# google/libultrahdr

Hardware: AMD Instinct MI355X
Metric: Mpixels/s encode+decode (API-1 P010+YUV420, 4K), device-resident round trip (higher is better)
Workload: dtype f32; 1 GPU; API-1 3840x2160 round trip per step: encode (P010 HLG + YCbCr420 -> two-pass 3-ch gain map at scale 1, FDCT q95, Huffman: two JPEG scans) + decode (Huffman, IDCT, applyGainMap -> RGBA_F16 linear); frames resident in HBM

## Files before the change

### libultrahdr_amd/csrc/api_context.cpp

```cpp
#include "api_internal.h"

#include <sys/mman.h>
#include <mutex>
#include <algorithm>

namespace uhdr_api {
uhdr_error_info_t ensure(DeviceBuf& b, size_t bytes) {
  if (b.cap >= bytes) return ok_status();
  if (b.p) (void)hipFree(b.p);
  b.p = nullptr;
  b.cap = 0;
  size_t want = bytes + (bytes >> 3) + 256;
  HIP_TRY(hipMalloc(&b.p, want));
  b.cap = want;
  return ok_status();
}


size_t bytes_per_sample(int fmt) {
  switch (fmt) {
    case UHDR_IMG_FMT_24bppYCbCrP010:
    case UHDR_IMG_FMT_30bppYCbCr444: return 2;
    case UHDR_IMG_FMT_24bppRGB888: return 3;
    case UHDR_IMG_FMT_32bppRGBA8888:
// ... 507 lines not shown
  int n = 0;
  if (hipGetDeviceCount(&n) != hipSuccess) return 0;
  return n;
}

int uhdr_hip_current_device(void) {
  int d = -1;
  if (hipGetDevice(&d) != hipSuccess) return -1;
  return d;
}

uhdr_hip_ctx_t* uhdr_hip_create(int device, uhdr_error_info_t* err) {
  auto fail = [&](const char* what, hipError_t e) -> uhdr_hip_ctx_t* {
    if (err) *err = err_status(UHDR_CODEC_ERROR, "uhdr_hip_create: %s failed: %s (no CPU fallback exists behind this library)",
                               what, hipGetErrorString(e));
    return nullptr;
  };
  if (err) *err = ok_status();
  int n = 0;
  hipError_t e = hipGetDeviceCount(&n);
  if (e != hipSuccess || n == 0) return fail("hipGetDeviceCount", e == hipSuccess ? hipErrorNoDevice : e);
  if (device < 0) {
    e = hipGetDevice(&device);
    if (e != hipSuccess) return fail("hipGetDevice", e);
  }
  if (device >= n) return fail("device index", hipErrorInvalidDevice);
  e = hipSetDevice(device);
  if (e != hipSuccess) return fail("hipSetDevice", e);
  uhdr_hip_ctx* c = new uhdr_hip_ctx();
  c->device = device;
  {
    const char* e = getenv("UHDR_HIP_HUFF_TWO_PASS");
    c->huff_two_pass = e && atoi(e) != 0;
    e = getenv("UHDR_HIP_HUFF_ROUTE_LOG");
    c->huff_route_log = e && atoi(e) != 0;
  }
  e = hipStreamCreateWithFlags(&c->own_stream, hipStreamNonBlocking);
  if (e != hipSuccess) { delete c; return fail("hipStreamCreate", e); }
  c->stream = c->own_stream;
  uhdr_error_info_t st = upload_lut(&c->d_srgb, host::srgb_inv_oetf_lut(), c->stream);
  if (st.error_code != UHDR_CODEC_OK) {
    if (err) *err = st;
    (void)hipStreamDestroy(c->own_stream);
    delete c;
    return nullptr;
  }
  return c;
}

void uhdr_hip_destroy(uhdr_hip_ctx_t* c) {
  if (!c) return;
  (void)hipSetDevice(c->device);
  (void)hipStreamSynchronize(c->stream);
  for (auto& e : c->prof_entries) { (void)hipEventDestroy(e.a); (void)hipEventDestroy(e.b); }
  float* luts[] = {c->d_srgb, c->d_hlg_inv, c->d_pq_inv, c->d_hlg_oetf, c->d_pq_oetf, c->d_hlg_inv_ootf, (float*)c->d_math,
                   c->d_hlg_buckets, c->d_pq_buckets, c->d_hlg_buckets_pre, c->d_pq_buckets_pre};
  for (float* p : luts) if (p) (void)hipFree(p);
  for (int i = 0; i < kTableSlots; i++) {
    if (c->h_tab[i]) (void)hipHostFree(c->h_tab[i]);
    if (c->d_tab[i]) (void)hipFree(c->d_tab[i]);
    if (c->tab_ev[i]) (void)hipEventDestroy(c->tab_ev[i]);
  }
  for (auto& b : c->scratch) if (b.p) (void)hipFree(b.p);
  for (auto& b : c->jpg) if (b.p) (void)hipFree(b.p);
  for (auto& b : c->enc) if (b.p) (void)hipFree(b.p);
  if (c->huff_slots.p) (void)hipFree(c->huff_slots.p);
// ... 274 lines not shown
```

### libultrahdr_amd/csrc/api_entropy.cpp

```cpp
#include "api_internal.h"

#include <condition_variable>
#include <functional>
#include <mutex>

uhdr_error_info_t uhdr_api::check_scan(const uhdr_hip_jpeg_scan_t* sc, bool need_coef, int* mcus_per_row, int* mcu_rows, int* blocks_per_mcu) {
  if (!sc) return err_status(UHDR_CODEC_INVALID_PARAM, "received nullptr for the scan description");
  if (sc->num_components != 1 && sc->num_components != 3)
    return err_status(UHDR_CODEC_INVALID_PARAM, "a scan has 1 or 3 components, received %d", sc->num_components);
  if (sc->w == 0 || sc->h == 0 || sc->w > 65535 || sc->h > 65535)
    return err_status(UHDR_CODEC_INVALID_PARAM, "image dimensions %ux%u are outside JPEG's 1..65535", sc->w, sc->h);
  int hmax = 1, vmax = 1, bpm = 0;
  for (int i = 0; i < sc->num_components; i++) {
    const int hs = sc->num_components == 1 ? 1 : sc->h_samp[i], vs = sc->num_components == 1 ? 1 : sc->v_samp[i];
    if (hs < 1 || hs > 2 || vs < 1 || vs > 2) return err_status(UHDR_CODEC_INVALID_PARAM, "component %d: sampling factors %dx%d not in {1, 2}", i, hs, vs);
    if (hs > hmax) hmax = hs;
    if (vs > vmax) vmax = vs;
    bpm += hs * vs;
    if (need_coef && (!sc->coef[i] || ((uintptr_t)sc->coef[i] & 15)))
      return err_status(UHDR_CODEC_INVALID_PARAM, "coefficient buffer %d is null or not 16-byte aligned", i);
    if (sc->blocks_w[i] < 1 || sc->blocks_h[i] < 1) return err_status(UHDR_CODEC_INVALID_PARAM, "component %d: empty block grid", i);
  }
  if (sc->num_components == 1) {
    *mcus_per_row = sc->blocks_w[0];
// ... 40 lines not shown
  const bool stream = sc->restart_interval == 0;
  if (!stream && (sc->restart_interval < 1 || sc->restart_interval > 65535 || sc->restart_interval * bpm > 64))
    return err_status(UHDR_CODEC_UNSUPPORTED_FEATURE, "restart_interval must be 0 (no markers) or in 1..%d for %d blocks per MCU (one wavefront "
                      "encodes one restart interval of at most 64 blocks); received %d", 64 / bpm, bpm, sc->restart_interval);
  if (stream && 2 * bpm > 64) return err_status(UHDR_CODEC_UNSUPPORTED_FEATURE, "%d blocks per MCU: outside the HIP path", bpm);
  HIP_TRY(hipSetDevice(c->device));
  if (!c->d_huff) {
    std::vector<uint32_t> blob(host::jpeg_huff_code_tables());
    blob.resize((size_t)host::kHuffTabWords + 16);
    memcpy(blob.data() + host::kHuffTabWords, host::jpeg_zigzag_to_natural(), 64);
    HIP_TRY(hipMalloc((void**)&c->d_huff, blob.size() * sizeof(uint32_t)));
    HIP_TRY(hipMemcpyAsync(c->d_huff, blob.data(), blob.size() * sizeof(uint32_t), hipMemcpyHostToDevice, c->stream));
    HIP_TRY(hipStreamSynchronize(c->stream));
  }
  HuffArgs a;
  memset(&a, 0, sizeof a);
  a.ncomp = sc->num_components;
  for (int i = 0; i < a.ncomp; i++) {
    a.coef[i] = sc->coef[i];
    a.bw[i] = sc->blocks_w[i]; a.bh[i] = sc->blocks_h[i];
    a.hs[i] = a.ncomp == 1 ? 1 : sc->h_samp[i]; a.vs[i] = a.ncomp == 1 ? 1 : sc->v_samp[i];
  }
  a.mcus_per_row = mpr;
  a.total_mcus = mpr * mrows;
  a.ri = stream ? huff_stream_segment_mcus(bpm) : sc->restart_interval;
  a.blocks_per_mcu = bpm;
  a.nseg = (a.total_mcus + a.ri - 1) / a.ri;
  a.tables = c->d_huff;
  a.zigzag = (const uint8_t*)(c->d_huff + host::kHuffTabWords);
  if (stream) {
    if (out_capacity > 0xFFFFFFF0u) out_capacity = 0xFFFFFFF0u;
    HuffStream t;
    memset(&t, 0, sizeof t);
    t.raw_words = ((uint64_t)out_capacity + 3) / 4 + 1;
    const uint64_t worst_words = (uint64_t)a.total_mcus * bpm * 52 + 2;
    if (t.raw_words > worst_words) t.raw_words = worst_words;
    const int nchunks = huff_stuff_chunks(t.raw_words * 4u);
    UHDR_TRY(ensure(c->scratch[4], (size_t)t.raw_words * 4));
    UHDR_TRY(ensure(c->scratch[5], ((size_t)a.nseg + 2) * sizeof(uint64_t) + (4 + (size_t)a.nseg + (size_t)nchunks) * sizeof(uint32_t)));
    t.raw = (uint32_t*)c->scratch[4].p;
    t.seg_start = (uint64_t*)c->scratch[5].p;
    uint64_t* d_total = t.seg_start + (size_t)a.nseg + 1;
    t.meta = (uint32_t*)(d_total + 1);
    t.seg_bits = t.meta + 4;
    uint32_t* chunk_counts = t.seg_bits + a.nseg;
    if (!c->huff_two_pass) {
      const size_t need = huff_stream_slot_bytes(a.nseg);
      if (c->huff_slots.cap >= need || !c->huff_slots_refused || need < c->huff_slots_refused) {
        if (ensure(c->huff_slots, need).error_code == UHDR_CODEC_OK) {
          t.slots = (uint32_t*)c->huff_slots.p;
        } else {
          (void)hipGetLastError();
          c->huff_slots_refused = need;
          fprintf(stderr, "uhdr_hip: no device memory for %zu bytes of Huffman segment slots: marker-less scans of that size take the two-pass route\n", need);
        }
      }
    }
    if (c->huff_route_log) fprintf(stderr, "uhdr_hip: huffman_encode stream route=%s nseg=%d\n", t.slots ? "one_walk" : "two_pass", a.nseg);
    {
      ProfScope ps(c, "huffman_encode");
      HIP_TRY(launch_huffman_encode_stream(a, t, chunk_counts, d_total, out, (uint64_t)out_capacity, c->stream));
    }
    c->stats.entropy_encode_stream++;
    if (!c->h_flags) HIP_TRY(hipHostMalloc((void**)&c->h_flags, 64 * sizeof(uint32_t), hipHostMallocDefault));
    uint32_t* hp = c->h_flags + 48;
    HIP_TRY(hipMemcpyAsync(hp, d_total, sizeof(uint64_t) + 4 * sizeof(uint32_t), hipMemcpyDeviceToHost, c->stream));
    HIP_TRY(wait_stream(c));
    uint64_t total = 0;
    uint32_t meta[4] = {0, 0, 0, 0};
    memcpy(&total, hp, sizeof total);
    memcpy(meta, hp + 2, sizeof meta);
    if (meta[2]) return err_status(UHDR_CODEC_INVALID_PARAM, "coefficients outside the baseline range (DC difference beyond 11 bits / AC beyond 10 bits)");
    const uint64_t raw_bytes = ((((uint64_t)meta[1] << 32) | meta[0]) + 7) / 8;
    if (raw_bytes > t.raw_words * 4u) total = raw_bytes + raw_bytes / 64 + 64;
    *out_bytes = (size_t)total;
    if (total > out_capacity)
      return err_status(UHDR_CODEC_MEM_ERROR, "entropy-coded data needs %llu bytes, the output buffer holds %zu", (unsigned long long)total, out_capacity);
    return ok_status();
  }
  a.slot_stride = huff_slot_stride();
  UHDR_TRY(ensure(c->scratch[4], (size_t)a.nseg * a.slot_stride));
  const size_t meta = (size_t)a.nseg * sizeof(uint32_t) + 16 + ((size_t)a.nseg + 1) * sizeof(uint64_t) + 16;
  UHDR_TRY(ensure(c->scratch[5], meta));
  a.slots = (uint8_t*)c->scratch[4].p;
  uint64_t* offsets = (uint64_t*)c->scratch[5].p;
  uint32_t* status = (uint32_t*)(offsets + (size_t)a.nseg + 1);
  a.seg_bytes = status + 2;
  {
    ProfScope ps(c, "huffman_encode");
    HIP_TRY(launch_huffman_encode(a, offsets, status, out, (uint64_t)out_capacity, c->stream));
  }
  c->stats.entropy_encode_intervals++;
  uint64_t total = 0;
  uint32_t bad = 0;
  HIP_TRY(hipMemcpyAsync(&total, offsets + a.nseg, sizeof total, hipMemcpyDeviceToHost, c->stream));
  HIP_TRY(hipMemcpyAsync(&bad, status, sizeof bad, hipMemcpyDeviceToHost, c->stream));
  HIP_TRY(wait_stream(c));
  if (bad) return err_status(UHDR_CODEC_INVALID_PARAM, "coefficients outside the baseline range (DC difference beyond 11 bits / AC beyond 10 bits)");
  *out_bytes = (size_t)total;
  if (total > out_capacity)
    return err_status(UHDR_CODEC_MEM_ERROR, "entropy-coded data needs %llu bytes, the output buffer holds %zu", (unsigned long long)total, out_capacity);
  return ok_status();
}

static bool make_dec_table(const uint8_t bits[17], const uint8_t vals[256], HuffDecTable* t) {
  memset(t, 0, sizeof *t);
  int nsym = 0;
// ... 554 lines not shown
  if (a.nseg == 1 && !c->huff_serial_ok && data_bytes > (256u << 10)) {
    c->stats.entropy_decode_declined++;
    return err_status(UHDR_CODEC_UNSUPPORTED_FEATURE, "a %zu-byte scan without restart markers that the parallel decoder does not take (Huffman tables outside its two-level form)", data_bytes);
  }
  if (!coef_zeroed)
    for (int i = 0; i < a.ncomp; i++) HIP_TRY(hipMemsetAsync(a.coef[i], 0, zero_bytes[i], c->stream));
  HIP_TRY(hipMemsetAsync(a.status, 0, 16, c->stream));
  {
    ProfScope ps(c, "huffman_decode");
    HIP_TRY(launch_huffman_decode(a, counts, starts, ends, c->stream));
  }
  if (a.nseg == 1) c->stats.entropy_decode_single_lane++;
  else c->stats.entropy_decode_intervals++;
  uint32_t st[2] = {0, 0};
  HIP_TRY(hipMemcpyAsync(st, a.status, sizeof st, hipMemcpyDeviceToHost, c->stream));
  HIP_TRY(wait_stream(c));
  if (st[1] != (uint32_t)(a.nseg - 1))
    return err_status(UHDR_CODEC_INVALID_PARAM, "found %u restart markers, a restart interval of %d MCUs over %d MCUs needs %d", st[1], a.ri,
                      a.total_mcus, a.nseg - 1);
  if (st[0] & 4u) return err_status(UHDR_CODEC_INVALID_PARAM, "restart markers out of sequence");
  if (st[0] & 2u) return err_status(UHDR_CODEC_INVALID_PARAM, "corrupt entropy-coded data (undefined Huffman code or a run past the end of a block)");
  return ok_status();
}

uhdr_error_info_t uhdr_api::aux_context(uhdr_hip_ctx* c, uhdr_hip_ctx** out) {
  if (!c->aux) {
    uhdr_error_info_t e = ok_status();
    c->aux = uhdr_hip_create(c->device, &e);
    if (!c->aux) return e.error_code != UHDR_CODEC_OK ? e : err_status(UHDR_CODEC_ERROR, "could not create the auxiliary context");
  }
  c->aux->prof = c->prof;
  c->aux->huff_serial_ok = c->huff_serial_ok;
  c->aux->huff_route_log = c->huff_route_log;
  c->aux->huff_two_pass = c->huff_two_pass;
  *out = c->aux;
  return ok_status();
}
void uhdr_api::aux_merge(uhdr_hip_ctx* c) {
  if (!c->aux) return;
  uhdr_hip_ctx* x = c->aux;
  c->stats.entropy_decode_parallel += x->stats.entropy_decode_parallel;
  c->stats.entropy_decode_intervals += x->stats.entropy_decode_intervals;
  c->stats.entropy_decode_single_lane += x->stats.entropy_decode_single_lane;
  c->stats.entropy_decode_declined += x->stats.entropy_decode_declined;
  c->stats.entropy_encode_stream += x->stats.entropy_encode_stream;
  c->stats.entropy_encode_intervals += x->stats.entropy_encode_intervals;
  x->stats = uhdr_hip_stats_t();
  for (auto& e : x->prof_entries) c->prof_entries.push_back(e);
  x->prof_entries.clear();
}

struct AuxWorker {
  static constexpr int kSpinUs = 300;
  std::thread th;
  std::mutex mu;
  std::condition_variable cv;
  std::function<void()> job;
  std::atomic<int> state{0};
  std::atomic<bool> busy{false};
  static bool spin_until(const std::function<bool()>& pred, int us) {
    const auto t0 = std::chrono::steady_clock::now();
    while (!pred()) {
      if (std::chrono::steady_clock::now() - t0 > std::chrono::microseconds(us)) return pred();
#if defined(__x86_64__)
      __builtin_ia32_pause();
#endif
// ... 129 lines not shown
```

### libultrahdr_amd/csrc/api_internal.h

```cpp
#ifndef UHDR_HIP_API_INTERNAL_H
#define UHDR_HIP_API_INTERNAL_H

#pragma GCC visibility push(default)
#include "uhdr_hip.h"
#pragma GCC visibility pop

#include <cfloat>
#include <chrono>
#include <cmath>
#include <cstdarg>
#include <cstdio>
#include <cstring>
#include <atomic>
#include <functional>
#include <map>
#include <memory>
#include <string>
#include <thread>
#include <vector>
#include "exact_math.h"
#include "host_tables.h"
#include "uhdr_types.h"
#include "rccl_bind.h"

// ... 46 lines not shown
constexpr int kTableSlots = 4;

struct DeviceBuf {
  void* p = nullptr;
  size_t cap = 0;
};

struct uhdr_hip_ctx {
  int device = 0;
  hipStream_t own_stream = nullptr;
  hipStream_t stream = nullptr;
  float* d_srgb = nullptr;
  float* d_hlg_inv = nullptr;
  float* d_pq_inv = nullptr;
  float* d_hlg_oetf = nullptr;
  float* d_pq_oetf = nullptr;
  float* d_hlg_buckets = nullptr;
  float* d_pq_buckets = nullptr;
  float* d_hlg_buckets_pre = nullptr;
  float* d_pq_buckets_pre = nullptr;
  float* d_hlg_inv_ootf = nullptr;
  double* d_math = nullptr;
  float* h_tab[kTableSlots] = {};
  float* d_tab[kTableSlots] = {};
  size_t tab_cap[kTableSlots] = {};
  hipEvent_t tab_ev[kTableSlots] = {};
  std::string tab_key[kTableSlots];
  int tab_next = 0;
  DeviceBuf scratch[8];
  uhdr_hip_stats_t stats = {};
  bool huff_serial_ok = true;
  DeviceBuf huff_slots;
  bool huff_two_pass = false;
  bool huff_route_log = false;
  size_t huff_slots_refused = 0;
  DeviceBuf enc[3];
  uhdr_hip_ctx* aux = nullptr;
  struct AuxWorker* aux_worker = nullptr;
  DeviceBuf jpg[6];
  struct Resident {
    DeviceBuf buf;
    bool valid = false;
    uhdr_img_fmt_t fmt = UHDR_IMG_FMT_UNSPECIFIED;
    unsigned int w = 0, h = 0;
    const void* host[3] = {};
    unsigned int host_stride[3] = {};
    size_t off[3] = {};
    unsigned int dev_stride[3] = {};
    unsigned int prows[3] = {}, pcols[3] = {};
    bool host_unwritten = false;
    bool adopted = false;
    void* adopt_dst = nullptr;
    unsigned int adopt_stride = 0, adopt_w = 0, adopt_h = 0;
    bool adopt_expand = false;
  } resident[2];
  struct HuffHint { uint32_t sub_bits = 0, bits_per_block = 0; } huff_hint[16];
  struct HuffTabCache {
    bool valid = false, fast_ok = false;
    uint8_t key[4 * (17 + 256)] = {};
    DeviceBuf dev;
  } huff_tabs;
  struct PinArena {
    void* p = nullptr;
    size_t cap = 0, off = 0;
    hipEvent_t ev = nullptr;
    bool ev_pending = false;
  } pin;
  uint32_t* h_flags = nullptr;
  bool resident_on = false;
  bool resident_lazy = false;
  uhdr_error_info_t sticky = {};
  unsigned int resident_next = 0;
  struct PendingCopy {
    DeviceBuf buf;
    bool on = false;
    size_t off = 0, pitch = 0, dst_pitch = 0;
    unsigned int w = 0, h = 0, bps = 0;
    bool expand = false;
    void* dst = nullptr;
    DeviceBuf tmp;
  } pending;
  struct MallEntry { const void* p; uint64_t stamp; };
  std::vector<MallEntry> mall;
  uint64_t mall_clock = 0;
  DeviceBuf minmax;
  uint32_t* d_huff = nullptr;
  CoefSrc* d_coef_src = nullptr;
  unsigned int coef_src_next = 0;
  CoefSrc* coef_src_last_slot = nullptr;
  std::vector<uint8_t> coef_src_last;
  float* d_srgb8 = nullptr;
  StepTab srgb8_meta = {};
  float* d_lin10[5] = {};
  struct GainTab { float mn, mx; float* d; StepTab meta; };
  std::vector<GainTab> gain_tabs;
  void* comm = nullptr;
  int comm_rank = 0, comm_size = 0;
  bool comm_custom = false;
  uhdr_hip_comm_ops_t comm_ops = {};
  DeviceBuf exchange;
// ... 82 lines not shown
```

### libultrahdr_amd/csrc/huffman_encode.hip

```cpp
#include "lds_copy.h"
#include "wg_scan.h"
#include "uhdr_types.h"

namespace uhdr {
namespace {

constexpr int kSegBlocks = 64;
constexpr int kWordsPerBlock = 52;
constexpr int kCoefRow = 33;

__device__ __forceinline__ uint32_t wave_incl_scan(uint32_t v, uint32_t lane) {
#pragma unroll
  for (int d = 1; d < 64; d <<= 1) {
    const uint32_t y = (uint32_t)__shfl_up((int)v, d, 64);
    if (lane >= (uint32_t)d) v += y;
  }
  return v;
}

__device__ __forceinline__ uint64_t zigzag_nonzero_map(const uint32_t* s_coef, uint32_t zz_of_lane, uint32_t lane) {
  uint64_t mine = 0;
  const uint32_t word = zz_of_lane >> 1, sh = (zz_of_lane & 1u) * 16u;
#pragma unroll 4
  for (uint32_t b = 0; b < (uint32_t)kSegBlocks; b++) {
// ... 342 lines not shown
          if (cnt >= 32u) {
            cnt -= 32u;
            atomicOr(&s_bits[w++], (uint32_t)(acc >> cnt));
          }
        });
        if (cnt) atomicOr(&s_bits[w], (uint32_t)(acc << (32u - cnt)));
      }
      __syncthreads();
      const uint64_t end_bit = start + total_bits;
      if (seg == a.nseg - 1 && lane == 0 && (end_bit & 7u)) {
        const uint32_t e = phase + total_bits, pad = 8u - (e & 7u), pos = e & 31u;
        s_bits[e >> 5] |= ((1u << pad) - 1u) << (32u - pos - pad);
      }
      __syncthreads();
      const uint64_t w0 = start >> 5;
      const uint32_t tail = (phase + total_bits) & 31u;
      for (uint32_t i = lane; i < nwords; i += 64) {
        if (w0 + i >= t.raw_words) break;
        const uint32_t v = __builtin_bswap32(s_bits[i]);
        const bool shared = (i == 0 && phase != 0) || (i == nwords - 1 && tail != 0);
        if (shared) atomicOr(&t.raw[w0 + i], v);
        else t.raw[w0 + i] = v;
      }
    }
  }
}

constexpr int kWalkSegs = 4;
constexpr int kSlotWords = kSegBlocks * kWordsSmall;
__device__ __forceinline__ void wave_sync() {
  __builtin_amdgcn_fence(__ATOMIC_SEQ_CST, "wavefront");
  __builtin_amdgcn_wave_barrier();
}
__global__ __launch_bounds__(64 * kWalkSegs) void huff_stream_walk_kernel(const HuffArgs a, const HuffStream t) {
  __shared__ __attribute__((aligned(16))) uint32_t s_tab[2 * (16 + 256)];
  __shared__ uint32_t s_coef_all[kWalkSegs][kSegBlocks * kCoefRow];
  __shared__ uint32_t s_bits_all[kWalkSegs][kSlotWords];
  __shared__ uint8_t s_zz[64];
  const uint32_t lane = threadIdx.x & 63u, wv = threadIdx.x >> 6;
  copy_words_to_lds<4>(s_tab, a.tables, 2 * (16 + 256), threadIdx.x, 64 * kWalkSegs);
  if (threadIdx.x < 64) s_zz[threadIdx.x] = a.zigzag[threadIdx.x];
  __syncthreads();
  uint32_t* s_coef = s_coef_all[wv];
  uint32_t* s_bits = s_bits_all[wv];
  const int bpm = a.blocks_per_mcu;
  const int mcu_local = (int)lane / bpm, k_in_mcu = (int)lane - mcu_local * bpm;
  int c = 0, kk = k_in_mcu;
  if (a.ncomp > 1) {
    while (c < a.ncomp - 1 && kk >= a.hs[c] * a.vs[c]) { kk -= a.hs[c] * a.vs[c]; c++; }
  }
  const int hs = a.ncomp > 1 ? a.hs[c] : 1, vs = a.ncomp > 1 ? a.vs[c] : 1;
  const int yi = kk / hs, xi = kk - yi * hs;
  const int pred_lane = (kk > 0 ? (int)lane - 1 : (int)lane - bpm + hs * vs - 1) & 63;
  const uint32_t* dct = s_tab + (c ? (16 + 256) : 0);
  const uint32_t* act = dct + 16;
  const uint32_t zz_of_lane = s_zz[lane];
  uint32_t* crow = s_coef + lane * kCoefRow;
  for (int seg = (int)blockIdx.x * kWalkSegs + (int)wv; seg < a.nseg; seg += (int)gridDim.x * kWalkSegs) {
    wave_sync();
    const int mcu = seg * a.ri + mcu_local - 1;
    const bool valid = mcu_local <= a.ri && mcu >= 0 && mcu < a.total_mcus;
    const bool emits = valid && mcu_local >= 1;
    const int mcu_c = valid ? mcu : 0;
    const int my = mcu_c / a.mcus_per_row, mx = mcu_c - my * a.mcus_per_row;
    const int by = my * vs + yi, bx = mx * hs + xi;
    const bool real = valid && by < a.bh[c] && bx < a.bw[c];
// ... 19 lines not shown
      else if (k_in_mcu >= 2 && ((real_mask >> (lane - 2)) & 1ull)) dcv = up2;
      else if (k_in_mcu >= 3 && ((real_mask >> (lane - 3)) & 1ull)) dcv = up3;
    }
    const int pred_v = __shfl(dcv, pred_lane, 64);
    const int diff = dcv - (emits ? pred_v : 0);
    wave_sync();
    const uint64_t nz = zigzag_nonzero_map(s_coef, zz_of_lane, lane);
    uint32_t len = 0, oob = 0;
    if (emits) walk_block(dct, act, diff, real, crow, s_zz, nz, oob, [&](uint32_t, uint32_t n) { len += n; });
    const uint32_t incl = wave_incl_scan(len, lane);
    const uint32_t total_bits = (uint32_t)__shfl((int)incl, 63, 64);
    const bool bad = __builtin_amdgcn_ballot_w64(oob != 0) != 0;
    if (lane == 0) t.seg_bits[seg] = bad ? kBadCoef : total_bits;
    if (bad || total_bits + 32u > (uint32_t)kSlotWords * 32u) continue;
    const uint32_t nwords = (total_bits + 31u) >> 5;
    for (uint32_t i = lane; i < nwords + 1u; i += 64) s_bits[i] = 0u;
    wave_sync();
    if (emits) {
      const uint32_t off = incl - len;
      uint64_t acc = 0;
      uint32_t cnt = off & 31u, w = off >> 5;
      walk_block(dct, act, diff, real, crow, s_zz, nz, oob, [&](uint32_t code, uint32_t n) {
        acc = (acc << n) | (uint64_t)code;
        cnt += n;
        if (cnt >= 32u) {
          cnt -= 32u;
          atomicOr(&s_bits[w++], (uint32_t)(acc >> cnt));
        }
      });
      if (cnt) atomicOr(&s_bits[w], (uint32_t)(acc << (32u - cnt)));
    }
    wave_sync();
    uint32_t* slot = t.slots + (size_t)seg * (size_t)kSlotWords;
    for (uint32_t i = lane; i < nwords; i += 64) slot[i] = s_bits[i];
  }
}

constexpr int kPlaceSegs = 4;
__global__ __launch_bounds__(64 * kPlaceSegs) void huff_stream_place_kernel(int nseg, const HuffStream t) {
  const uint32_t lane = threadIdx.x & 63u;
  const int seg = (int)blockIdx.x * kPlaceSegs + (int)(threadIdx.x >> 6);
  if (seg >= nseg) return;
  const uint32_t total_bits = t.seg_bits[seg];
  if (total_bits >= kRetry || total_bits + 32u > (uint32_t)(kSegBlocks * kWordsSmall) * 32u) return;
  const uint64_t start = t.seg_start[seg];
  const uint32_t phase = (uint32_t)(start & 31u);
  const uint32_t nin = (total_bits + 31u) >> 5, nwords = (phase + total_bits + 31u) >> 5;
  const uint32_t e = phase + total_bits, tail = e & 31u;
  const bool flush = seg == nseg - 1 && (e & 7u);
  const uint32_t* slot = t.slots + (size_t)seg * (size_t)(kSegBlocks * kWordsSmall);
  const uint64_t w0 = start >> 5;
  for (uint32_t i = lane; i < nwords; i += 64) {
    if (w0 + i >= t.raw_words) break;
    const uint32_t cur = i < nin ? slot[i] : 0u, prev = (i > 0 && phase != 0) ? slot[i - 1] : 0u;
    uint32_t v = __builtin_amdgcn_alignbit(prev, cur, phase);
    if (flush && i == (e >> 5)) {
      const uint32_t pad = 8u - (e & 7u);
      v |= ((1u << pad) - 1u) << (32u - tail - pad);
    }
    v = __builtin_bswap32(v);
    const bool shared = (i == 0 && phase != 0) || (i == nwords - 1 && tail != 0);
    if (shared) atomicOr(&t.raw[w0 + i], v);
    else t.raw[w0 + i] = v;
  }
}

template <int NT = 1024, typename Sink>
// ... 26 lines not shown
}

constexpr int kStreamScanThreads = 256;
__global__ __launch_bounds__(kStreamScanThreads) void huff_stream_scan_kernel(const uint32_t* __restrict__ seg_bits, int nseg, const HuffStream t) {
  __shared__ uint32_t s_val[8 * kStreamScanThreads];
  __shared__ uint64_t s_sum[kStreamScanThreads / 64];
  __shared__ uint32_t s_bad;
  const int tid = (int)threadIdx.x;
  if (tid == 0) s_bad = 0;
  __syncthreads();
  bool bad = false;
  uint32_t big = 0;
  const uint64_t total = wg_scan_tiles<kStreamScanThreads>(seg_bits, nseg, s_val, s_sum, [&](int i, uint32_t n, uint64_t run) {
    bad |= n >= kRetry;
    big += (n < kRetry && n + 32u > (uint32_t)(kSegBlocks * kWordsSmall) * 32u) ? 1u : 0u;
    t.seg_start[i] = run;
    if ((run >> 5) < t.raw_words) t.raw[run >> 5] = 0u;
  });
  if (bad) atomicOr(&s_bad, 1u);
  if (big) atomicAdd(&s_bad, big << 1);
  __syncthreads();
  if (tid == kStreamScanThreads - 1) {
    t.seg_start[nseg] = total;
    if ((total >> 5) < t.raw_words) t.raw[total >> 5] = 0u;
    t.meta[0] = (uint32_t)total;
    t.meta[1] = (uint32_t)(total >> 32);
  }
  if (tid == 0) {
    t.meta[2] = s_bad & 1u;
    t.meta[3] = s_bad >> 1;
  }
}

__device__ __forceinline__ uint32_t ff_mask16(const uint4& v, uint32_t nv) {
  const uint32_t w[4] = {v.x, v.y, v.z, v.w};
  uint32_t m = 0;
#pragma unroll
  for (uint32_t k = 0; k < 16; k++) m |= (k < nv && ((w[k >> 2] >> (8u * (k & 3u))) & 0xffu) == 0xffu) ? (1u << k) : 0u;
  return m;
}
__device__ __forceinline__ uint4 raw_load16(const HuffStream& t, uint64_t base) {
  const uint64_t w = base >> 2;
  if (w + 4u <= t.raw_words) return *(const uint4*)(t.raw + w);
  uint32_t x[4] = {0, 0, 0, 0};
  for (uint32_t k = 0; k < 4; k++)
    if (w + k < t.raw_words) x[k] = t.raw[w + k];
  return make_uint4(x[0], x[1], x[2], x[3]);
}
__global__ __launch_bounds__(256) void huff_stuff_count_kernel(const HuffStream t, uint32_t* __restrict__ counts) {
  __shared__ uint32_t s_n;
  const uint64_t total_bits = (uint64_t)t.meta[0] | ((uint64_t)t.meta[1] << 32);
  const uint64_t nraw = (total_bits + 7u) >> 3;
  const uint64_t base = (uint64_t)blockIdx.x * kStuffChunk + threadIdx.x * 16u;
  if ((uint64_t)blockIdx.x * kStuffChunk >= nraw) {
    if (threadIdx.x == 0) counts[blockIdx.x] = 0;
    return;
  }
  if (threadIdx.x == 0) s_n = 0;
  __syncthreads();
  uint32_t n = 0;
  if (base < nraw) n = (uint32_t)__builtin_popcount(ff_mask16(raw_load16(t, base), (uint32_t)min((uint64_t)16, nraw - base)));
  n = wave_incl_scan(n, threadIdx.x & 63);
  if ((threadIdx.x & 63) == 63 && n) atomicAdd(&s_n, n);
  __syncthreads();
  if (threadIdx.x == 0) counts[blockIdx.x] = s_n;
}
// ... 38 lines not shown
  }
  const uint32_t w[4] = {v.x, v.y, v.z, v.w};
  for (uint32_t k = 0; k < nv; k++) {
    const uint32_t b = (w[k >> 2] >> (8u * (k & 3u))) & 0xffu;
    if (pos < cap) out[pos] = (uint8_t)b;
    pos++;
    if (b == 0xffu) {
      if (pos < cap) out[pos] = 0;
      pos++;
    }
  }
}

}

uint32_t huff_slot_stride() { return (uint32_t)(kSegBlocks * kWordsPerBlock * 4 * 2); }

hipError_t launch_huffman_encode(const HuffArgs& a, uint64_t* offsets, uint32_t* status, uint8_t* out, uint64_t cap, hipStream_t s) {
  int grid = a.nseg < 8192 ? a.nseg : 8192;
  const int per = a.ri * a.blocks_per_mcu, groups = per > 32 ? 1 : 64 / per;
  const int nwseg = (a.nseg + groups - 1) / groups;
  hipLaunchKernelGGL((huff_encode_kernel<kWordsSmall, false>), dim3(nwseg < 8192 ? nwseg : 8192), dim3(64), 0, s, a);
  hipLaunchKernelGGL((huff_encode_kernel<kWordsPerBlock, true>), dim3(grid < 2048 ? grid : 2048), dim3(64), 0, s, a);
  hipLaunchKernelGGL(huff_offsets_kernel, dim3(1), dim3(1024), 0, s, a.seg_bytes, a.nseg, offsets, status);
  hipLaunchKernelGGL(huff_gather_kernel, dim3(grid), dim3(256), 0, s, a.slots, a.slot_stride, a.seg_bytes, offsets, a.nseg, out, cap);
  return hipGetLastError();
}


int huff_stream_segment_mcus(int blocks_per_mcu) { return kSegBlocks / blocks_per_mcu - 1; }
size_t huff_stream_slot_bytes(int nseg) { return (size_t)nseg * (size_t)kSlotWords * sizeof(uint32_t); }
int huff_stuff_chunks(uint64_t raw_bytes) { return (int)((raw_bytes + kStuffChunk - 1) / kStuffChunk); }

hipError_t launch_huffman_encode_stream(const HuffArgs& a, const HuffStream& t, uint32_t* chunk_counts, uint64_t* out_bytes, uint8_t* out, uint64_t cap,
                                        hipStream_t s) {
  const int grid = a.nseg < 16384 ? a.nseg : 16384;
  const int nchunks = huff_stuff_chunks(t.raw_words * 4u);
  if (t.slots) {
    const int wgrid = (grid + kWalkSegs - 1) / kWalkSegs;
    hipLaunchKernelGGL(huff_stream_walk_kernel, dim3(wgrid), dim3(64 * kWalkSegs), 0, s, a, t);
    hipLaunchKernelGGL(huff_stream_scan_kernel, dim3(1), dim3(kStreamScanThreads), 0, s, (const uint32_t*)t.seg_bits, a.nseg, t);
    hipLaunchKernelGGL(huff_stream_place_kernel, dim3((a.nseg + kPlaceSegs - 1) / kPlaceSegs), dim3(64 * kPlaceSegs), 0, s, a.nseg, t);
  } else {
    hipLaunchKernelGGL((huff_stream_kernel<1, 0>), dim3(grid), dim3(64), 0, s, a, t);
    hipLaunchKernelGGL(huff_stream_scan_kernel, dim3(1), dim3(kStreamScanThreads), 0, s, (const uint32_t*)t.seg_bits, a.nseg, t);
    hipLaunchKernelGGL((huff_stream_kernel<kWordsSmall, 1>), dim3(grid), dim3(64), 0, s, a, t);
  }
  hipLaunchKernelGGL((huff_stream_kernel<kWordsPerBlock, 2>), dim3(grid < 2048 ? grid : 2048), dim3(64), 0, s, a, t);
  hipLaunchKernelGGL(huff_stuff_count_kernel, dim3(nchunks), dim3(256), 0, s, t, chunk_counts);
  hipLaunchKernelGGL(huff_stuff_scan_kernel, dim3(1), dim3(kStreamScanThreads), 0, s, chunk_counts, nchunks, t, out_bytes);
  hipLaunchKernelGGL(huff_stuff_scatter_kernel, dim3(nchunks), dim3(256), 0, s, t, (const uint32_t*)chunk_counts, out, cap);
  return hipGetLastError();
}

}
```

### libultrahdr_amd/csrc/uhdr_types.h

```cpp
#pragma once
#include <hip/hip_runtime.h>
#include <stdint.h>

#include "device_math.h"
#include "uhdr_hip.h"

namespace uhdr {

struct ImageView {
  const void* p[3];
  uint32_t stride[3];
  uint32_t w, h;
  int fmt;
  int range;
};
struct ImageViewMut {
  void* p[3];
  uint32_t stride[3];
  uint32_t w, h;
  int fmt;
  int range;
};

constexpr int kSrgbN = 1024;
// ... 222 lines not shown
struct ResizePlane {
  const void* src;
  void* dst;
  uint32_t src_w, src_h, dst_w;
  uint32_t rows, y0;
  size_t src_pitch, dst_pitch;
  double scale_x, scale_y;
};
hipError_t launch_resize_image(const ResizePlane& p, int bpp, hipStream_t s);

struct HuffArgs {
  const int16_t* coef[3];
  int bw[3], bh[3];
  int hs[3], vs[3];
  int ncomp;
  int mcus_per_row, total_mcus;
  int ri;
  int blocks_per_mcu;
  int nseg;
  const uint32_t* tables;
  const uint8_t* zigzag;
  uint8_t* slots;
  uint32_t slot_stride;
  uint32_t* seg_bytes;
};
uint32_t huff_slot_stride();
struct HuffStream {
  uint32_t* seg_bits;
  uint64_t* seg_start;
  uint32_t* raw;
  uint64_t raw_words;
  uint32_t* meta;
  uint32_t* slots;
};
int huff_stream_segment_mcus(int blocks_per_mcu);
size_t huff_stream_slot_bytes(int nseg);
int huff_stuff_chunks(uint64_t raw_bytes);
hipError_t launch_huffman_encode_stream(const HuffArgs& a, const HuffStream& t, uint32_t* chunk_counts, uint64_t* out_bytes, uint8_t* out, uint64_t cap,
                                        hipStream_t s);
hipError_t launch_huffman_encode(const HuffArgs& a, uint64_t* offsets, uint32_t* status, uint8_t* out, uint64_t cap, hipStream_t s);

struct HuffDecTable {
  uint16_t lut[512];
  int maxcode[18];
  int valoff[17];
  uint8_t vals[256];
};
struct HuffDecArgs {
  const uint8_t* data;
  uint32_t nbytes;
  const uint32_t* starts;
  const uint32_t* ends;
  int nseg, ri, total_mcus, mcus_per_row, ncomp;
  int bw[3], bh[3], hs[3], vs[3];
  int16_t* coef[3];
  const HuffDecTable* tabs;
  const uint8_t* zigzag;
  uint32_t* status;
};
constexpr int kHuffL2Max = 16;
struct HuffFastTable {
  uint16_t l1[512];
  uint16_t l2[kHuffL2Max][128];
};
constexpr int kHuffValWords = 512 + kHuffL2Max * 128;
constexpr int kHuffPairBits = 10, kHuffPairWords = 1 << kHuffPairBits;
constexpr int kHuffL2Total = 32;
constexpr int kHuffPairBlobWords = 4 * kHuffPairWords + kHuffL2Total * 128 / 2;
constexpr int kHuffPairValBlobWords = 8 * kHuffPairWords + kHuffL2Total * 128 / 2;
struct HuffSyncArgs {
  const uint8_t* clean;
  uint32_t nbytes;
// ... 79 lines not shown
```

Measured before the change: 12700 Mpixels/s.

## Place Huffman segments directly into stuffed output, skipping raw-stream tail

The walk kernel now also counts 0xFF bytes at each of the eight possible bit alignments and records each segment's edge bits. A new single-block scan derives the bit offsets and a byte-stuffing prefix, and a new place kernel writes the stuffed bytes straight into the output. This drops the raw intermediate stream and the three stuffing kernels (count, scan, scatter). The result is written into host-mapped pinned memory, so the extra D2H memcpy is gone. Oversized segments fall back to the old raw-stream tail, which costs another sync and launch round, and the stuffing arithmetic at segment boundaries is intricate and could have edge-case bugs.

```diff
diff --git a/libultrahdr_amd/csrc/api_context.cpp b/libultrahdr_amd/csrc/api_context.cpp
--- a/libultrahdr_amd/csrc/api_context.cpp
+++ b/libultrahdr_amd/csrc/api_context.cpp
@@ -563,6 +563,8 @@
   {
     const char* e = getenv("UHDR_HIP_HUFF_TWO_PASS");
     c->huff_two_pass = e && atoi(e) != 0;
+    e = getenv("UHDR_HIP_HUFF_RAW_TAIL");
+    c->huff_raw_tail = e && atoi(e) != 0;
     e = getenv("UHDR_HIP_HUFF_ROUTE_LOG");
     c->huff_route_log = e && atoi(e) != 0;
   }
diff --git a/libultrahdr_amd/csrc/api_entropy.cpp b/libultrahdr_amd/csrc/api_entropy.cpp
--- a/libultrahdr_amd/csrc/api_entropy.cpp
+++ b/libultrahdr_amd/csrc/api_entropy.cpp
@@ -96,13 +96,12 @@
     if (out_capacity > 0xFFFFFFF0u) out_capacity = 0xFFFFFFF0u;
     HuffStream t;
     memset(&t, 0, sizeof t);
-    t.raw_words = ((uint64_t)out_capacity + 3) / 4 + 1;
+    uint64_t raw_words = ((uint64_t)out_capacity + 3) / 4 + 1;
     const uint64_t worst_words = (uint64_t)a.total_mcus * bpm * 52 + 2;
-    if (t.raw_words > worst_words) t.raw_words = worst_words;
-    const int nchunks = huff_stuff_chunks(t.raw_words * 4u);
-    UHDR_TRY(ensure(c->scratch[4], (size_t)t.raw_words * 4));
-    UHDR_TRY(ensure(c->scratch[5], ((size_t)a.nseg + 2) * sizeof(uint64_t) + (4 + (size_t)a.nseg + (size_t)nchunks) * sizeof(uint32_t)));
-    t.raw = (uint32_t*)c->scratch[4].p;
+    if (raw_words > worst_words) raw_words = worst_words;
+    const int nchunks = huff_stuff_chunks(raw_words * 4u);
+    const size_t head = (((size_t)a.nseg + 2) * sizeof(uint64_t) + (4 + (size_t)a.nseg + (size_t)nchunks) * sizeof(uint32_t) + 15) & ~(size_t)15;
+    UHDR_TRY(ensure(c->scratch[5], head + (size_t)a.nseg * 6 * sizeof(uint32_t)));
     t.seg_start = (uint64_t*)c->scratch[5].p;
     uint64_t* d_total = t.seg_start + (size_t)a.nseg + 1;
     t.meta = (uint32_t*)(d_total + 1);
@@ -120,23 +119,53 @@
         }
       }
     }
-    if (c->huff_route_log) fprintf(stderr, "uhdr_hip: huffman_encode stream route=%s nseg=%d\n", t.slots ? "one_walk" : "two_pass", a.nseg);
+    if (!c->h_flags) HIP_TRY(hipHostMalloc((void**)&c->h_flags, 64 * sizeof(uint32_t), hipHostMallocDefault));
+    uint32_t* hp = c->h_flags + 48;
+    const bool direct = t.slots && !c->huff_raw_tail;
+    if (direct) {
+      if (!c->h_flags_dev) HIP_TRY(hipHostGetDevicePointer((void**)&c->h_flags_dev, c->h_flags, 0));
+      t.seg_ff = (uint32_t*)((uint8_t*)c->scratch[5].p + head);
+      t.seg_edge = t.seg_ff + (size_t)a.nseg * 4;
+      t.seg_zero = t.seg_edge + a.nseg;
+      t.result = c->h_flags_dev + 48;
+    }
+    auto raw_stream = [&]() -> uhdr_error_info_t {
+      UHDR_TRY(ensure(c->scratch[4], (size_t)raw_words * 4));
+      t.raw = (uint32_t*)c->scratch[4].p;
+      t.raw_words = raw_words;
+      return ok_status();
+    };
+    if (!direct) UHDR_TRY(raw_stream());
+    if (c->huff_route_log)
+      fprintf(stderr, "uhdr_hip: huffman_encode stream route=%s nseg=%d tail=%s\n", t.slots ? "one_walk" : "two_pass", a.nseg, direct ? "direct" : "raw");
     {
       ProfScope ps(c, "huffman_encode");
       HIP_TRY(launch_huffman_encode_stream(a, t, chunk_counts, d_total, out, (uint64_t)out_capacity, c->stream));
     }
     c->stats.entropy_encode_stream++;
-    if (!c->h_flags) HIP_TRY(hipHostMalloc((void**)&c->h_flags, 64 * sizeof(uint32_t), hipHostMallocDefault));
-    uint32_t* hp = c->h_flags + 48;
-    HIP_TRY(hipMemcpyAsync(hp, d_total, sizeof(uint64_t) + 4 * sizeof(uint32_t), hipMemcpyDeviceToHost, c->stream));
-    HIP_TRY(wait_stream(c));
     uint64_t total = 0;
     uint32_t meta[4] = {0, 0, 0, 0};
-    memcpy(&total, hp, sizeof total);
-    memcpy(meta, hp + 2, sizeof meta);
+    auto read_back = [&](bool copy) -> uhdr_error_info_t {
+      if (copy) HIP_TRY(hipMemcpyAsync(hp, d_total, sizeof(uint64_t) + 4 * sizeof(uint32_t), hipMemcpyDeviceToHost, c->stream));
+      HIP_TRY(wait_stream(c));
+      memcpy(&total, hp, sizeof total);
+      memcpy(meta, hp + 2, sizeof meta);
+      return ok_status();
+    };
+    UHDR_TRY(read_back(!direct));
     if (meta[2]) return err_status(UHDR_CODEC_INVALID_PARAM, "coefficients outside the baseline range (DC difference beyond 11 bits / AC beyond 10 bits)");
+    bool raw_tail = !direct;
+    if (direct && meta[3]) {
+      UHDR_TRY(raw_stream());
+      {
+        ProfScope ps(c, "huffman_encode");
+        HIP_TRY(launch_huffman_encode_stream_tail(a, t, chunk_counts, d_total, out, (uint64_t)out_capacity, c->stream));
+      }
+      UHDR_TRY(read_back(true));
+      raw_tail = true;
+    }
     const uint64_t raw_bytes = ((((uint64_t)meta[1] << 32) | meta[0]) + 7) / 8;
-    if (raw_bytes > t.raw_words * 4u) total = raw_bytes + raw_bytes / 64 + 64;
+    if (raw_tail && raw_bytes > t.raw_words * 4u) total = raw_bytes + raw_bytes / 64 + 64;
     *out_bytes = (size_t)total;
     if (total > out_capacity)
       return err_status(UHDR_CODEC_MEM_ERROR, "entropy-coded data needs %llu bytes, the output buffer holds %zu", (unsigned long long)total, out_capacity);
@@ -757,6 +786,7 @@
   c->aux->prof = c->prof;
   c->aux->huff_serial_ok = c->huff_serial_ok;
   c->aux->huff_route_log = c->huff_route_log;
+  c->aux->huff_raw_tail = c->huff_raw_tail;
   c->aux->huff_two_pass = c->huff_two_pass;
   *out = c->aux;
   return ok_status();
diff --git a/libultrahdr_amd/csrc/api_internal.h b/libultrahdr_amd/csrc/api_internal.h
--- a/libultrahdr_amd/csrc/api_internal.h
+++ b/libultrahdr_amd/csrc/api_internal.h
@@ -102,6 +102,7 @@
   bool huff_serial_ok = true;
   DeviceBuf huff_slots;
   bool huff_two_pass = false;
+  bool huff_raw_tail = false;
   bool huff_route_log = false;
   size_t huff_slots_refused = 0;
   DeviceBuf enc[3];
@@ -136,6 +137,7 @@
     hipEvent_t ev = nullptr;
     bool ev_pending = false;
   } pin;
+  uint32_t* h_flags_dev = nullptr;
   uint32_t* h_flags = nullptr;
   bool resident_on = false;
   bool resident_lazy = false;
diff --git a/libultrahdr_amd/csrc/huffman_encode.hip b/libultrahdr_amd/csrc/huffman_encode.hip
--- a/libultrahdr_amd/csrc/huffman_encode.hip
+++ b/libultrahdr_amd/csrc/huffman_encode.hip
@@ -398,6 +398,12 @@
   __builtin_amdgcn_fence(__ATOMIC_SEQ_CST, "wavefront");
   __builtin_amdgcn_wave_barrier();
 }
+__device__ __forceinline__ uint32_t ff_bytes(uint32_t v, int nv) {
+  const uint32_t valid = nv >= 4 ? 0xFFFFFFFFu : nv <= 0 ? 0u : ~(0xFFFFFFFFu >> (8 * nv));
+  const uint32_t y = ~(v & valid);
+  return ~(((y & 0x7F7F7F7Fu) + 0x7F7F7F7Fu) | y | 0x7F7F7F7Fu);
+}
+template <bool DIRECT>
 __global__ __launch_bounds__(64 * kWalkSegs) void huff_stream_walk_kernel(const HuffArgs a, const HuffStream t) {
   __shared__ __attribute__((aligned(16))) uint32_t s_tab[2 * (16 + 256)];
   __shared__ uint32_t s_coef_all[kWalkSegs][kSegBlocks * kCoefRow];
@@ -483,7 +489,36 @@
     }
     wave_sync();
     uint32_t* slot = t.slots + (size_t)seg * (size_t)kSlotWords;
-    for (uint32_t i = lane; i < nwords; i += 64) slot[i] = s_bits[i];
+    if constexpr (!DIRECT) {
+      for (uint32_t i = lane; i < nwords; i += 64) slot[i] = s_bits[i];
+    } else {
+      uint32_t cnt2[4] = {0, 0, 0, 0};
+      for (uint32_t i = lane; i < nwords; i += 64) {
+        const uint32_t hi = s_bits[i], lo = s_bits[i + 1];
+        slot[i] = hi;
+        const int left = (int)total_bits - (int)(32u * i);
+#pragma unroll
+        for (int r = 0; r < 8; r++) {
+          const int d = (8 - r) & 7;
+          const uint32_t v = d ? __builtin_amdgcn_alignbit(hi, lo, (uint32_t)(32 - d)) : hi;
+          cnt2[r >> 1] += (uint32_t)__builtin_popcount(ff_bytes(v, (left - d) >> 3)) << (16 * (r & 1));
+        }
+      }
+#pragma unroll
+      for (int k = 0; k < 4; k++) {
+#pragma unroll
+        for (int d = 32; d >= 1; d >>= 1) cnt2[k] += (uint32_t)__shfl_xor((int)cnt2[k], d, 64);
+      }
+      if (lane == 0) {
+        const uint32_t lead = min((uint32_t)__clz((int)~s_bits[0]), 8u);
+        const uint32_t ew = total_bits >> 5, es = total_bits & 31u;
+        const uint32_t whi = ew ? s_bits[ew - 1] : 0u, wlo = s_bits[ew];
+        const uint32_t win = es ? __builtin_amdgcn_alignbit(whi, wlo, 32u - es) : whi;
+        const uint32_t trail = min((uint32_t)__builtin_ctz(~win | 0x100u), 8u);
+        *(uint4*)(t.seg_ff + (size_t)seg * 4) = make_uint4(cnt2[0], cnt2[1], cnt2[2], cnt2[3]);
+        t.seg_edge[seg] = lead | (trail << 8);
+      }
+    }
   }
 }
 
@@ -576,6 +611,164 @@
   }
 }
 
+constexpr int kDirectTile = 8 * kStreamScanThreads;
+__global__ __launch_bounds__(kStreamScanThreads) void huff_stream_scan_direct_kernel(int nseg, const HuffStream t) {
+  constexpr int NT = kStreamScanThreads;
+  __shared__ uint32_t s_val[8 * NT];
+  __shared__ uint64_t s_sum[NT / 64];
+  __shared__ uint32_t s_bad;
+  const int tid = (int)threadIdx.x;
+  if (tid == 0) s_bad = 0;
+  __syncthreads();
+  bool bad = false;
+  uint32_t big = 0;
+  uint64_t carry_bits = 0, carry_ff = 0;
+  const uint4* ffrec = (const uint4*)t.seg_ff;
+  for (int base = 0; base < nseg; base += kDirectTile) {
+    uint32_t b[8], bn[8], ed[8], edn[8];
+    uint4 rec[8];
+#pragma unroll
+    for (int j = 0; j < 8; j++) {
+      const int e0 = min(base + j * NT + tid, nseg - 1), e1 = min(base + j * NT + tid + 1, nseg - 1);
+      b[j] = t.seg_bits[e0];
+      bn[j] = t.seg_bits[e1];
+      ed[j] = t.seg_edge[e0];
+      edn[j] = t.seg_edge[e1];
+      rec[j] = ffrec[e0];
+    }
+#pragma unroll
+    for (int j = 0; j < 8; j++) s_val[j * NT + tid] = base + j * NT + tid < nseg ? b[j] : 0u;
+    __syncthreads();
+    uint32_t x[8];
+    uint64_t sum = 0;
+#pragma unroll
+    for (int j = 0; j < 8; j++) { x[j] = s_val[tid * 8 + j]; sum += x[j]; }
+    uint64_t sc[1] = {sum}, all[1];
+    wg_incl_scan<NT, 1>(sc, s_sum, all);
+    uint64_t run = carry_bits + sc[0] - sum;
+#pragma unroll
+    for (int j = 0; j < 8; j++) {
+      const int i = base + tid * 8 + j;
+      if (i < nseg) {
+        bad |= x[j] >= kRetry;
+        big += (x[j] < kRetry && x[j] + 32u > (uint32_t)kSlotWords * 32u) ? 1u : 0u;
+        t.seg_start[i] = run;
+      }
+      s_val[tid * 8 + j] = (uint32_t)run & 7u;
+      run += x[j];
+    }
+    carry_bits += all[0];
+    __syncthreads();
+    uint32_t f[8];
+#pragma unroll
+    for (int j = 0; j < 8; j++) {
+      const int e = base + j * NT + tid;
+      const uint32_t r = s_val[j * NT + tid];
+      const uint32_t w = r < 2 ? rec[j].x : r < 4 ? rec[j].y : r < 6 ? rec[j].z : rec[j].w;
+      uint32_t n = (w >> (16u * (r & 1u))) & 0xffffu;
+      const uint32_t m = (r + b[j]) & 7u;
+      if (m != 0 && b[j] >= m && ((ed[j] >> 8) & 0xffu) >= m) {
+        uint32_t need = 8u - m;
+        if (e + 1 == nseg - 1) need = min(need, bn[j]);
+        if (e == nseg - 1 || (edn[j] & 0xffu) >= need) n++;
+      }
+      f[j] = e < nseg ? n : 0u;
+    }
+    __syncthreads();
+#pragma unroll
+    for (int j = 0; j < 8; j++) s_val[j * NT + tid] = f[j];
+    __syncthreads();
+    sum = 0;
+#pragma unroll
+    for (int j = 0; j < 8; j++) { x[j] = s_val[tid * 8 + j]; sum += x[j]; }
+    sc[0] = sum;
+    wg_incl_scan<NT, 1>(sc, s_sum, all);
+    run = carry_ff + sc[0] - sum;
+#pragma unroll
+    for (int j = 0; j < 8; j++) {
+      const int i = base + tid * 8 + j;
+      if (i < nseg) t.seg_zero[i] = (uint32_t)run;
+      run += x[j];
+    }
+    carry_ff += all[0];
+  }
+  if (bad) atomicOr(&s_bad, 1u);
+  if (big) atomicAdd(&s_bad, big << 1);
+  __syncthreads();
+  if (tid == NT - 1) {
+    t.seg_start[nseg] = carry_bits;
+    const uint64_t stuffed = ((carry_bits + 7u) >> 3) + carry_ff;
+    t.meta[0] = (uint32_t)carry_bits;
+    t.meta[1] = (uint32_t)(carry_bits >> 32);
+    t.result[0] = (uint32_t)stuffed;
+    t.result[1] = (uint32_t)(stuffed >> 32);
+    t.result[2] = (uint32_t)carry_bits;
+    t.result[3] = (uint32_t)(carry_bits >> 32);
+  }
+  if (tid == 0) {
+    const uint32_t sb = s_bad;
+    t.meta[2] = sb & 1u;
+    t.meta[3] = sb >> 1;
+    t.result[4] = sb & 1u;
+    t.result[5] = sb >> 1;
+  }
+}
+
+__global__ __launch_bounds__(64 * kPlaceSegs) void huff_stream_place_direct_kernel(int nseg, const HuffStream t, uint8_t* __restrict__ out, uint64_t cap) {
+  if (t.meta[2] | t.meta[3]) return;
+  const uint32_t lane = threadIdx.x & 63u;
+  const int seg = (int)blockIdx.x * kPlaceSegs + (int)(threadIdx.x >> 6);
+  if (seg >= nseg) return;
+  const uint32_t B = t.seg_bits[seg];
+  if (B + 32u > (uint32_t)kSlotWords * 32u) return;
+  const uint64_t S = t.seg_start[seg];
+  const uint64_t j0 = (S + 7u) >> 3;
+  const uint32_t nown = (uint32_t)(((S + B + 7u) >> 3) - j0);
+  if (nown == 0) return;
+  const uint32_t d = (8u - ((uint32_t)S & 7u)) & 7u;
+  const uint32_t nin = (B + 31u) >> 5;
+  const uint32_t* slot = t.slots + (size_t)seg * (size_t)kSlotWords;
+  uint32_t nxt = 0xFFFFFFFFu;
+  if (seg + 1 < nseg) {
+    nxt = slot[kSlotWords];
+    const uint32_t bn = t.seg_bits[seg + 1];
+    if (seg + 1 == nseg - 1 && bn < 32u) nxt |= 0xFFFFFFFFu >> bn;
+  }
+  const uint32_t qb = B >> 5, sb = B & 31u;
+  auto word = [&](uint32_t q, uint32_t v) -> uint32_t {
+    uint32_t x = q < nin ? v : 0u;
+    if (q == qb) x |= nxt >> sb;
+    if (q == qb + 1u && sb != 0u) x |= nxt << (32u - sb);
+    return x;
+  };
+  uint64_t pos0 = j0 + t.seg_zero[seg];
+  for (uint32_t q0 = 0; 4u * q0 < nown; q0 += 64) {
+    const uint32_t q = q0 + lane;
+    const uint32_t a0 = slot[min(q, nin - 1u)], a1 = slot[min(q + 1u, nin - 1u)];
+    const uint32_t hi = word(q, a0), lo = word(q + 1u, a1);
+    const uint32_t v = d ? __builtin_amdgcn_alignbit(hi, lo, 32u - d) : hi;
+    const int nv = (int)nown - (int)(4u * q);
+    const uint32_t mask = ff_bytes(v, nv), nff = (uint32_t)__builtin_popcount(mask);
+    const uint32_t incl = wave_incl_scan(nff, lane);
+    uint64_t pos = pos0 + 4u * lane + (incl - nff);
+    if (nff == 0 && nv >= 4 && pos + 4u <= cap) {
+      const uint32_t le = __builtin_bswap32(v);
+      __builtin_memcpy(out + pos, &le, 4);
+    } else {
+      for (int k = 0; k < 4 && k < nv; k++) {
+        const uint32_t byte = (v >> (24 - 8 * k)) & 0xffu;
+        if (pos < cap) out[pos] = (uint8_t)byte;
+        pos++;
+        if (byte == 0xffu) {
+          if (pos < cap) out[pos] = 0;
+          pos++;
+        }
+      }
+    }
+    pos0 += 256u + (uint32_t)__shfl((int)incl, 63, 64);
+  }
+}
+
 __device__ __forceinline__ uint32_t ff_mask16(const uint4& v, uint32_t nv) {
   const uint32_t w[4] = {v.x, v.y, v.z, v.w};
   uint32_t m = 0;
@@ -680,20 +873,13 @@
 size_t huff_stream_slot_bytes(int nseg) { return (size_t)nseg * (size_t)kSlotWords * sizeof(uint32_t); }
 int huff_stuff_chunks(uint64_t raw_bytes) { return (int)((raw_bytes + kStuffChunk - 1) / kStuffChunk); }
 
-hipError_t launch_huffman_encode_stream(const HuffArgs& a, const HuffStream& t, uint32_t* chunk_counts, uint64_t* out_bytes, uint8_t* out, uint64_t cap,
-                                        hipStream_t s) {
+hipError_t launch_huffman_encode_stream_tail(const HuffArgs& a, const HuffStream& t, uint32_t* chunk_counts, uint64_t* out_bytes, uint8_t* out,
+                                             uint64_t cap, hipStream_t s) {
   const int grid = a.nseg < 16384 ? a.nseg : 16384;
   const int nchunks = huff_stuff_chunks(t.raw_words * 4u);
-  if (t.slots) {
-    const int wgrid = (grid + kWalkSegs - 1) / kWalkSegs;
-    hipLaunchKernelGGL(huff_stream_walk_kernel, dim3(wgrid), dim3(64 * kWalkSegs), 0, s, a, t);
-    hipLaunchKernelGGL(huff_stream_scan_kernel, dim3(1), dim3(kStreamScanThreads), 0, s, (const uint32_t*)t.seg_bits, a.nseg, t);
-    hipLaunchKernelGGL(huff_stream_place_kernel, dim3((a.nseg + kPlaceSegs - 1) / kPlaceSegs), dim3(64 * kPlaceSegs), 0, s, a.nseg, t);
-  } else {
-    hipLaunchKernelGGL((huff_stream_kernel<1, 0>), dim3(grid), dim3(64), 0, s, a, t);
-    hipLaunchKernelGGL(huff_stream_scan_kernel, dim3(1), dim3(kStreamScanThreads), 0, s, (const uint32_t*)t.seg_bits, a.nseg, t);
-    hipLaunchKernelGGL((huff_stream_kernel<kWordsSmall, 1>), dim3(grid), dim3(64), 0, s, a, t);
-  }
+  hipLaunchKernelGGL(huff_stream_scan_kernel, dim3(1), dim3(kStreamScanThreads), 0, s, (const uint32_t*)t.seg_bits, a.nseg, t);
+  if (t.slots) hipLaunchKernelGGL(huff_stream_place_kernel, dim3((a.nseg + kPlaceSegs - 1) / kPlaceSegs), dim3(64 * kPlaceSegs), 0, s, a.nseg, t);
+  else hipLaunchKernelGGL((huff_stream_kernel<kWordsSmall, 1>), dim3(grid), dim3(64), 0, s, a, t);
   hipLaunchKernelGGL((huff_stream_kernel<kWordsPerBlock, 2>), dim3(grid < 2048 ? grid : 2048), dim3(64), 0, s, a, t);
   hipLaunchKernelGGL(huff_stuff_count_kernel, dim3(nchunks), dim3(256), 0, s, t, chunk_counts);
   hipLaunchKernelGGL(huff_stuff_scan_kernel, dim3(1), dim3(kStreamScanThreads), 0, s, chunk_counts, nchunks, t, out_bytes);
@@ -701,4 +887,19 @@
   return hipGetLastError();
 }
 
-}
+hipError_t launch_huffman_encode_stream(const HuffArgs& a, const HuffStream& t, uint32_t* chunk_counts, uint64_t* out_bytes, uint8_t* out, uint64_t cap,
+                                        hipStream_t s) {
+  const int grid = a.nseg < 16384 ? a.nseg : 16384;
+  const int wgrid = (grid + kWalkSegs - 1) / kWalkSegs;
+  if (t.slots && t.seg_ff) {
+    hipLaunchKernelGGL(huff_stream_walk_kernel<true>, dim3(wgrid), dim3(64 * kWalkSegs), 0, s, a, t);
+    hipLaunchKernelGGL(huff_stream_scan_direct_kernel, dim3(1), dim3(kStreamScanThreads), 0, s, a.nseg, t);
+    hipLaunchKernelGGL(huff_stream_place_direct_kernel, dim3((a.nseg + kPlaceSegs - 1) / kPlaceSegs), dim3(64 * kPlaceSegs), 0, s, a.nseg, t, out, cap);
+    return hipGetLastError();
+  }
+  if (t.slots) hipLaunchKernelGGL(huff_stream_walk_kernel<false>, dim3(wgrid), dim3(64 * kWalkSegs), 0, s, a, t);
+  else hipLaunchKernelGGL((huff_stream_kernel<1, 0>), dim3(grid), dim3(64), 0, s, a, t);
+  return launch_huffman_encode_stream_tail(a, t, chunk_counts, out_bytes, out, cap, s);
+}
+
+}
diff --git a/libultrahdr_amd/csrc/uhdr_types.h b/libultrahdr_amd/csrc/uhdr_types.h
--- a/libultrahdr_amd/csrc/uhdr_types.h
+++ b/libultrahdr_amd/csrc/uhdr_types.h
@@ -278,12 +278,18 @@
   uint64_t raw_words;
   uint32_t* meta;
   uint32_t* slots;
+  uint32_t* seg_ff;
+  uint32_t* seg_edge;
+  uint32_t* seg_zero;
+  uint32_t* result;
 };
 int huff_stream_segment_mcus(int blocks_per_mcu);
 size_t huff_stream_slot_bytes(int nseg);
 int huff_stuff_chunks(uint64_t raw_bytes);
 hipError_t launch_huffman_encode_stream(const HuffArgs& a, const HuffStream& t, uint32_t* chunk_counts, uint64_t* out_bytes, uint8_t* out, uint64_t cap,
                                         hipStream_t s);
+hipError_t launch_huffman_encode_stream_tail(const HuffArgs& a, const HuffStream& t, uint32_t* chunk_counts, uint64_t* out_bytes, uint8_t* out, uint64_t cap,
+                                             hipStream_t s);
 hipError_t launch_huffman_encode(const HuffArgs& a, uint64_t* offsets, uint32_t* status, uint8_t* out, uint64_t cap, hipStream_t s);
 
 struct HuffDecTable {
```

Result: no change. 12780 Mpixels/s, median of 4 (+0.6%).
